# HSG-AIML/MaskedSST

Measured on NVIDIA B200. Metric: simmim_pretrain_samples_per_sec, higher is better.
Workload: dtype bf16

## Files before the change

### maskedsst_b200/csrc/attn_block_tc.cu

```cuda
#include "common.cuh"
#include "kernels.h"
#include "attn_geom.cuh"
#include "ptx.cuh"
#include <stdlib.h>
#include <stdio.h>
#include <type_traits>

namespace msst {
using namespace ptx;
typedef __nv_bfloat16 bf16;
int make_tmap_bf16_nd(CUtensorMap* m, const void* base, int rank, const int64_t* dims, const int64_t* strides, const int* box, int swizzle_bytes);
int make_tmap_nd(CUtensorMap* m, const void* base, int elem_bytes, int rank, const int64_t* dims, const int64_t* strides, const int* box, int swizzle_bytes);

namespace {

constexpr int AB_THREADS = 608;
constexpr int AB_MAXR = 8;
constexpr uint32_t AB_T16 = 16384;
constexpr uint32_t AB_BLK = 8192;
constexpr uint32_t COL_P = 0, COL_S = 192, COL_O = 256, COL_X = 192, COL_DH = 384;
constexpr uint32_t COL_Y = 320, Y_COLS = 96;

struct AbParams {
    AttnGeom g;
// ... 27 lines not shown
__device__ __forceinline__ uint64_t pair_base(const AttnGeom& g, int64_t group, int h) {
    return ((uint64_t)group * g.H + h) * (uint64_t)(TS * TS / 2);
}
__device__ __forceinline__ void group_coords(const AttnGeom& g, int64_t group, int& c1, int& c2, int& c3) {
    if (g.gpb == 0) { c1 = 0; c2 = (int)(group * g.G); c3 = 0; }
    else { c1 = (int)(group % g.gpb) * g.G; c2 = 0; c3 = (int)(group / g.gpb); }
}
__device__ __forceinline__ void store_row16(uint8_t* tile, int row, int cq, const uint32_t (&v)[16]) {
    uint8_t* r = tile + row * 128;
    const uint32_t sw = (uint32_t)(row & 7);
    *reinterpret_cast<uint4*>(r + ((((uint32_t)(2 * cq)) ^ sw) << 4)) =
        make_uint4(pack_bf(__uint_as_float(v[0]), __uint_as_float(v[1])), pack_bf(__uint_as_float(v[2]), __uint_as_float(v[3])),
                   pack_bf(__uint_as_float(v[4]), __uint_as_float(v[5])), pack_bf(__uint_as_float(v[6]), __uint_as_float(v[7])));
    *reinterpret_cast<uint4*>(r + ((((uint32_t)(2 * cq + 1)) ^ sw) << 4)) =
        make_uint4(pack_bf(__uint_as_float(v[8]), __uint_as_float(v[9])), pack_bf(__uint_as_float(v[10]), __uint_as_float(v[11])),
                   pack_bf(__uint_as_float(v[12]), __uint_as_float(v[13])), pack_bf(__uint_as_float(v[14]), __uint_as_float(v[15])));
}
__device__ __forceinline__ void store_row16_packed(uint8_t* tile, int row, int cq, const uint32_t (&pk)[8]) {
    uint8_t* r = tile + row * 128;
    const uint32_t sw = (uint32_t)(row & 7);
    *reinterpret_cast<uint4*>(r + ((((uint32_t)(2 * cq)) ^ sw) << 4)) = make_uint4(pk[0], pk[1], pk[2], pk[3]);
    *reinterpret_cast<uint4*>(r + ((((uint32_t)(2 * cq + 1)) ^ sw) << 4)) = make_uint4(pk[4], pk[5], pk[6], pk[7]);
}
__device__ __forceinline__ uint32_t key_mask16(const AttnGeom& g, int m, int cq) {
    uint32_t vm = 0;
    const int used = g.G * g.N;
    for (int j = 0; j < 16; ++j) {
        const int c = 16 * cq + j;
        const bool same = g.gpb == 0 ? (c / g.N == m / g.N) : (c % g.G == m % g.G);
        vm |= (uint32_t)(same && c < used && m < used) << j;
    }
    return vm;
}

struct alignas(8) AbBars {
    uint64_t h_full[2], h_empty[2], w_full[AB_MAXR], w_empty[AB_MAXR], do_full[2], do_empty[2];
    uint64_t pro_full, conv_done, s_full, sdp_read, p_full, o_full, a_ready, dh_full, dh_free, stg_full, stg_free, dhs_full, dhs_free;
    uint64_t y_full[2], out_full, out_free, xin_full, t_kfree[2], t_vfree[2], kv_free[2];
    uint32_t tmem_base;
};

struct AbCommon {
    uint8_t *h_s, *w_s;
    AbBars* bars;
    uint32_t tmem, h_addr, w_addr;
};
__device__ __forceinline__ void warp_arrive(uint64_t* bar, int lane) {
    __syncwarp();
    if (lane == 0) mbar_arrive(bar);
}
struct Ring {
    int slot; uint32_t ph; int NR;
    __device__ __forceinline__ void next() { if (++slot == NR) { slot = 0; ph ^= 1u; } }
};
constexpr uint64_t kDescHiK128 = ((uint64_t)(1024 >> 4) << 32) | (1ull << 46) | (kLayoutSW128 << 61);
__device__ __forceinline__ uint64_t kdesc(uint32_t addr) { return kDescHiK128 | (1ull << 16) | (uint64_t)((addr >> 4) & 0x3FFF); }
__device__ __forceinline__ uint64_t mndesc(uint32_t addr) { return kDescHiK128 | ((uint64_t)(AB_BLK >> 4) << 16) | (uint64_t)((addr >> 4) & 0x3FFF); }

template <int NCH>
__device__ __forceinline__ void load_h_tile(const AbParams& p, const CUtensorMap* tma_h, uint8_t* dst, uint64_t* bar, int64_t tile) {
    const AttnGeom& g = p.g;
    const uint32_t rows = p.nbox == 1 ? 128u : (uint32_t)(g.G * g.N);
    mbar_arrive_expect_tx(bar, (uint32_t)NCH * (uint32_t)p.nbox * rows * 64u);
    if (p.nbox == 1) {
#pragma unroll
        for (int c = 0; c < NCH; ++c) tma_load_2d(dst + c * 8192, tma_h, bar, c * 32, (int)(tile * 128));
    } else {
        for (int gi = 0; gi < 2; ++gi) {
            int c1, c2, c3;
            group_coords(g, tile * 2 + gi, c1, c2, c3);
#pragma unroll
            for (int c = 0; c < NCH; ++c) tma_load_4d(dst + c * 8192 + gi * 4096, tma_h, bar, c * 32, c1, c2, c3);
        }
    }
}
template <int NCH>
__device__ __forceinline__ void prefetch_h_tile(const AbParams& p, const CUtensorMap* tma_h, int64_t tile) {
    if (p.nbox == 1) {
#pragma unroll
        for (int c = 0; c < NCH; ++c) tma_prefetch_l2_2d(tma_h, c * 32, (int)(tile * 128));
    } else {
        for (int gi = 0; gi < 2; ++gi) {
            int c1, c2, c3;
            group_coords(p.g, tile * 2 + gi, c1, c2, c3);
#pragma unroll
            for (int c = 0; c < NCH; ++c) tma_prefetch_l2_4d(tma_h, c * 32, c1, c2, c3);
        }
    }
}
template <int NCH>
__device__ __forceinline__ void load_w_slice(const AbParams& p, const CUtensorMap* tma_w, AbBars* bars, uint8_t* w_s, Ring& r, int t, int h) {
    mbar_wait(&bars->w_empty[r.slot], r.ph ^ 1u);
    mbar_arrive_expect_tx(&bars->w_full[r.slot], (uint32_t)NCH * 4096u);
    uint8_t* dst = w_s + (size_t)r.slot * p.slot_bytes;
#pragma unroll
    for (int c = 0; c < NCH; ++c) tma_load_2d(dst + c * 4096, tma_w, &bars->w_full[r.slot], c * 32, t * p.g.H * 64 + h * 64);
    r.next();
}
template <int NCH>
__device__ __forceinline__ void issue_prologue(const AbParams& p, const AbCommon& s, int64_t k, int h, Ring& r, bool lead) {
    const int buf = (int)(k & 1);
    if (h == 0) mbar_wait(&s.bars->h_full[buf], (uint32_t)(k >> 1) & 1);
    const uint64_t ha = make_smem_desc_sw64(s.h_addr + (uint32_t)buf * p.hbuf_bytes);
    const uint32_t idesc = make_idesc_bf16(128, 64, 0, 0);
#pragma unroll
    for (int t = 0; t < 3; ++t) {
        mbar_wait(&s.bars->w_full[r.slot], r.ph);
        tc_fence_after();
        const uint64_t wa = make_smem_desc_sw64(s.w_addr + (uint32_t)r.slot * p.slot_bytes);
#pragma unroll
        for (int ks = 0; ks < 2 * NCH; ++ks)
            if (lead) umma_bf16(s.tmem + COL_P + 64 * t, ha + (uint64_t)(((ks >> 1) * 8192 + (ks & 1) * 32) >> 4), wa + (uint64_t)(((ks >> 1) * 4096 + (ks & 1) * 32) >> 4),
                      idesc, ks != 0);
        if (lead) umma_commit(&s.bars->w_empty[r.slot]);
        r.next();
    }
    if (lead && h == p.g.H - 1) umma_commit(&s.bars->h_empty[buf]);
    if (lead) umma_commit(&s.bars->pro_full);
}
template <int NCH>
__device__ __forceinline__ void issue_prologue_bwd(const AbParams& p, const AbCommon& s, int64_t k, int h, Ring& r, bool lead) {
    if (h == 0) mbar_wait(&s.bars->h_full[0], (uint32_t)k & 1);
    const uint64_t ha = make_smem_desc_sw64(s.h_addr);
    const uint32_t idesc = make_idesc_bf16(128, 64, 0, 1);
#pragma unroll
    for (int t = 0; t < 3; ++t) {
        mbar_wait(&s.bars->w_full[r.slot], r.ph);
        tc_fence_after();
        const uint64_t wa = mndesc(s.w_addr + (uint32_t)r.slot * p.slot_bytes);
#pragma unroll
        for (int ks = 0; ks < 2 * NCH; ++ks)
            if (lead) umma_bf16(s.tmem + COL_P + 64 * t, ha + (uint64_t)(((ks >> 1) * 8192 + (ks & 1) * 32) >> 4), wa + (uint64_t)(ks * 128), idesc, ks != 0);
        if (lead) umma_commit(&s.bars->w_empty[r.slot]);
        r.next();
    }
// ... 48 lines not shown
}
__device__ __forceinline__ void store_tile(const AbParams& p, const CUtensorMap* tm, const uint8_t* src, int col0, int64_t tile) {
    store_tile_rows(p, tm, src, 128, col0, tile);
}

constexpr int AB_THREADS_OUT = 736;
__device__ __forceinline__ void tail_load_x(const AbParams& p, AbBars* bars, const CUtensorMap* tma_x, uint8_t* dst, int c, int64_t tile) {
    const AttnGeom& g = p.g;
    const uint32_t rows = p.nbox == 1 ? 128u : (uint32_t)(g.G * g.N);
    mbar_arrive_expect_tx(&bars->xin_full, (uint32_t)p.nbox * rows * 128u);
    if (p.nbox == 1) tma_load_2d(dst, tma_x, &bars->xin_full, c * 32, (int)(tile * 128));
    else
        for (int gi = 0; gi < 2; ++gi) {
            int c1, c2, c3;
            group_coords(g, tile * 2 + gi, c1, c2, c3);
            tma_load_4d(dst + gi * AB_BLK, tma_x, &bars->xin_full, c * 32, c1, c2, c3);
        }
}
__device__ __forceinline__ void tail_prefetch_x(const AbParams& p, const CUtensorMap* tma_x, int c, int64_t tile) {
    if (tile >= p.n_tiles) return;
    if (p.nbox == 1) tma_prefetch_l2_2d(tma_x, c * 32, (int)(tile * 128));
    else
        for (int gi = 0; gi < 2; ++gi) {
            int c1, c2, c3;
            group_coords(p.g, tile * 2 + gi, c1, c2, c3);
            tma_prefetch_l2_4d(tma_x, c * 32, c1, c2, c3);
        }
}
__device__ __forceinline__ void tail_schedule(int h, int H, int nch, int& lo, int& hi) {
    lo = h; hi = (h == H - 1) ? nch : h;
    if (hi > nch) hi = nch;
}

template <int NCH, bool OUT>
__global__ void __launch_bounds__(OUT ? AB_THREADS_OUT : AB_THREADS, 1)
attn_block_fwd_kernel(const __grid_constant__ CUtensorMap tma_h, const __grid_constant__ CUtensorMap tma_w, const __grid_constant__ CUtensorMap tma_o,
                      const __grid_constant__ CUtensorMap tma_wo, const __grid_constant__ CUtensorMap tma_xmid, const __grid_constant__ CUtensorMap tma_h2,
                      const __grid_constant__ CUtensorMap tma_x, const __grid_constant__ AbParams p) {
    extern __shared__ __align__(1024) uint8_t smem_raw[];
    uint8_t* smem = smem_raw;
    if (smem_u32(smem) & 1023u) __trap();
    const AttnGeom& g = p.g;
    AbCommon s;
    s.h_s = smem; s.w_s = s.h_s + 2 * p.hbuf_bytes;
    uint8_t* qkv_s = s.w_s + (size_t)p.NR * p.slot_bytes;
    uint8_t* p_s = qkv_s + 6 * AB_T16;
    float* xch = reinterpret_cast<float*>(p_s + AB_T16);
    s.bars = reinterpret_cast<AbBars*>(xch + 2 * 4 * 128);
    AbBars* bars = s.bars;
    const int warp = threadIdx.x >> 5;
    const int H = g.H;
    constexpr int D = NCH * 32;
    ab_setup(bars, warp, s.h_s, 2 * p.hbuf_bytes, nullptr, 0, &tma_h, &tma_w, &tma_o, OUT ? &tma_wo : nullptr, OUT ? &tma_xmid : nullptr, OUT ? 2u : 1u);
    s.tmem = bars->tmem_base; s.h_addr = smem_u32(s.h_s); s.w_addr = smem_u32(s.w_s);

    const int64_t my_tiles = blockIdx.x < p.n_tiles ? (p.n_tiles - 1 - blockIdx.x) / gridDim.x + 1 : 0;
    const int64_t n_items = my_tiles * H;
    if (warp < 16) {
        const int lq = warp & 3, cq = warp >> 2, lane = threadIdx.x & 31;
        const int L = lq * 32 + lane;
        const uint32_t lane_addr = (uint32_t)(lq * 32) << 16;
        const int slot = 64 * ((lane >> 4) & 1) + 16 * lq + (lane & 15);
        const int blk = slot >> 6, m = slot & 63;
        const float sl2 = g.scale * 1.4426950408889634f;
        const bool full_blocks = g.N == 64 && g.groups % 2 == 0;
        const uint64_t seed = p.drop.seed + (p.drop.seed_dev ? __ldg(p.drop.seed_dev) : 0ull);
        const uint32_t t16 = p.drop.thresh >> 16;
        const uint32_t vm_geom = full_blocks ? 0xFFFFu : key_mask16(g, m, cq);
        float* xmax = xch; float* xsum = xch + 4 * 128;
        int64_t cur_tile = -1, grow = -1; uint32_t vm = 0;
        int64_t k = 0; int h = 0;
        bool hosted = false; uint32_t n_kvf0 = 0, n_kvf1 = 0;
        if (n_items > 0) {
            mbar_wait(&bars->pro_full, 0);
            tc_fence_after();
            convert_qkv(s.tmem, qkv_s, lane_addr, L, cq);
            tc_fence_before();
            fence_proxy_async();
            warp_arrive(&bars->conv_done, lane);
        }
        for (int64_t it = 0; it < n_items; ++it) {
            const uint32_t ph = (uint32_t)it & 1;
            const int64_t tile = blockIdx.x + k * gridDim.x;
            if (tile != cur_tile) {
                cur_tile = tile;
                int64_t seq; int pos;
                const int64_t group = tile * 2 + blk;
                const bool ok = group < g.groups && slot_to(g, group, 0, m, seq, pos);
                grow = ok ? row_of(g, seq, pos) : -1;
                vm = ok ? vm_geom : 0u;
            }
            const uint64_t hidx = pair_base(g, tile * 2 + blk, h) + (uint64_t)(m * 32 + 8 * cq);
            const uint32_t hash_lo = (uint32_t)hidx + (uint32_t)(seed >> 32);
            const uint32_t hash_hi = ((uint32_t)(hidx >> 32) * 0x85EBCA77u) ^ (uint32_t)seed ^ (p.drop.site * 0xC2B2AE3Du);
            if (threadIdx.x == 0) AB_T(it, 0);
            mbar_wait(&bars->s_full, ph);
            if (threadIdx.x == 0) AB_T(it, 1);
            tc_fence_after();
            float sc[16];
            {
                uint32_t a[16];
                tmem_ld_32x16(s.tmem + lane_addr + COL_S + 16 * cq, a);
                tmem_ld_wait();
#pragma unroll
                for (int j = 0; j < 16; ++j) sc[j] = __uint_as_float(a[j]);
            }
            float mx = -INFINITY;
            if (vm == 0xFFFFu) {
#pragma unroll
                for (int j = 0; j < 16; ++j) mx = fmaxf(mx, sc[j]);
            } else {
#pragma unroll
                for (int j = 0; j < 16; ++j) { sc[j] = (vm >> j) & 1u ? sc[j] : -INFINITY; mx = fmaxf(mx, sc[j]); }
            }
            xmax[cq * 128 + L] = mx;
            asm volatile("bar.sync 1, 512;" ::: "memory");
            mx = fmaxf(fmaxf(xmax[L], xmax[128 + L]), fmaxf(xmax[256 + L], xmax[384 + L]));
            const float sub = mx == -INFINITY ? 0.f : mx * sl2;
            float l = 0.f;
            uint32_t pk[8];
            auto exp_row = [&](auto drop_tag) {
                constexpr bool DROP = decltype(drop_tag)::value;
#pragma unroll
                for (int jj = 0; jj < 8; ++jj) {
                    float p0 = ex2_approx(fmaf(sc[2 * jj], sl2, -sub)), p1 = ex2_approx(fmaf(sc[2 * jj + 1], sl2, -sub));
                    l += p0 + p1;
                    if (DROP) {
                        uint32_t x = (hash_lo + (uint32_t)jj) * 0x9E3779B1u ^ hash_hi;
                        x ^= x >> 16; x *= 0x7feb352du; x ^= x >> 15; x *= 0x846ca68bu; x ^= x >> 16;
                        p0 *= (x & 0xFFFFu) >= t16 ? p.drop.scale : 0.f;
                        p1 *= (x >> 16) >= t16 ? p.drop.scale : 0.f;
                    }
                    pk[jj] = pack_bf(p0, p1);
                }
            };
            if (p.drop.on()) exp_row(std::true_type{}); else exp_row(std::false_type{});
            xsum[cq * 128 + L] = l;
            store_row16_packed(p_s + blk * AB_BLK, m, cq, pk);
            fence_proxy_async();
            tc_fence_before();
            warp_arrive(&bars->p_full, lane);
            if (threadIdx.x == 0) AB_T(it, 2);
            asm volatile("bar.sync 1, 512;" ::: "memory");
            l = (xsum[L] + xsum[128 + L]) + (xsum[256 + L] + xsum[384 + L]);
            const float inv = l > 0.f ? 1.f / l : 0.f;
            if (cq == 0 && grow >= 0) p.lse_out[grow * H + h] = (sub + log2f(l)) * 0.6931471805599453f;
            if (it >= 1) mbar_wait(&bars->stg_free, (uint32_t)(it - 1) & 1);
            if (it + 1 < n_items) {
                if (OUT && hosted) {
                    if (it & 1) { mbar_wait(&bars->kv_free[0], n_kvf0 & 1u); ++n_kvf0; }
                    else { mbar_wait(&bars->kv_free[1], n_kvf1 & 1u); ++n_kvf1; }
                }
                mbar_wait(&bars->pro_full, ph ^ 1u);
                if (threadIdx.x == 0) AB_T(it, 3);
                tc_fence_after();
                convert_qkv(s.tmem, qkv_s + (size_t)((it + 1) & 1) * 3 * AB_T16, lane_addr, L, cq);
                tc_fence_before();
                fence_proxy_async();
                warp_arrive(&bars->conv_done, lane);
                if (threadIdx.x == 0) AB_T(it, 4);
            }
            mbar_wait(&bars->o_full, ph);
            if (threadIdx.x == 0) AB_T(it, 5);
            tc_fence_after();
            {
                uint32_t v[16], o8[8];
                tmem_ld_32x16(s.tmem + lane_addr + COL_O + 16 * cq, v);
                tmem_ld_wait();
#pragma unroll
                for (int j = 0; j < 8; ++j) o8[j] = pack_bf(__uint_as_float(v[2 * j]) * inv, __uint_as_float(v[2 * j + 1]) * inv);
                store_row16_packed(qkv_s + (size_t)(it & 1) * 3 * AB_T16, slot, cq, o8);
            }
            tc_fence_before();
            fence_proxy_async();
            warp_arrive(&bars->stg_full, lane);
            if (threadIdx.x == 0) AB_T(it, 6);
            if (OUT) { int lo, hi; tail_schedule(h, H, NCH, lo, hi); hosted = k > 0 && lo <= hi; }
            if (++h == H) { h = 0; ++k; }
        }
    } else
    if (warp >= 16 && warp < 19) {
    if (warp == 16) {
        if (elect_one()) {
            Ring r{0, 0u, p.NR};
            int64_t pk = 0; int phd = 0;
            auto load_pro = [&]() {
                if (phd == 0) {
                    const int buf = (int)(pk & 1);
                    mbar_wait(&bars->h_empty[buf], ((uint32_t)(pk >> 1) & 1) ^ 1);
                    load_h_tile<NCH>(p, &tma_h, s.h_s + (size_t)buf * p.hbuf_bytes, &bars->h_full[buf], blockIdx.x + pk * gridDim.x);
                }
                for (int t = 0; t < 3; ++t) load_w_slice<NCH>(p, &tma_w, bars, s.w_s, r, t, phd);
                if (++phd == H) { phd = 0; ++pk; }
            };
            int yh = 0;
            auto load_wo = [&]() {
                mbar_wait(&bars->w_empty[r.slot], r.ph ^ 1u);
                mbar_arrive_expect_tx(&bars->w_full[r.slot], (uint32_t)D * 128u);
                tma_load_2d(s.w_s + (size_t)r.slot * p.slot_bytes, &tma_wo, &bars->w_full[r.slot], yh * 64, 0);
                r.next();
                if (++yh == H) yh = 0;
            };
            if (n_items > 0) load_pro();
            if (n_items > 1) load_pro();
            for (int64_t it = 0; it < n_items; ++it) {
                if (OUT && it >= 1) load_wo();
                if (it + 2 < n_items) load_pro();
            }
            if (OUT && n_items > 0) load_wo();
        }
    } else if (warp == 17) {
        if (n_items > 0) {
            const bool lead = elect_one();
            Ring r{0, 0u, p.NR};
            const uint32_t idesc_s = make_idesc_bf16(64, 64, 0, 0), idesc_o = make_idesc_bf16(64, 64, 0, 1), idesc_y = make_idesc_bf16(128, D, 0, 0);
            const uint32_t qkv_addr = smem_u32(qkv_s);
            const uint64_t pd0 = kdesc(smem_u32(p_s)), pd1 = kdesc(smem_u32(p_s) + AB_BLK);
            int64_t pk = 0; int phd = 0;
            auto next_pro = [&]() { issue_prologue<NCH>(p, s, pk, phd, r, lead); if (++phd == H) { phd = 0; ++pk; } };
            int64_t sk = 0; int sh = 0;
            auto issue_s = [&](int64_t it) {
                const uint32_t qa = qkv_addr + (uint32_t)(it & 1) * 3 * AB_T16;
                mbar_wait(&bars->conv_done, (uint32_t)it & 1);
                if (lead) AB_T(it, 8);
                tc_fence_after();
#pragma unroll
                for (int b = 0; b < 2; ++b) {
                    const uint64_t dq = kdesc(qa + b * AB_BLK), dk = kdesc(qa + AB_T16 + b * AB_BLK);
#pragma unroll
                    for (int ks = 0; ks < 4; ++ks)
                        if (lead) umma_bf16(s.tmem + COL_S + ((uint32_t)(16 * b) << 16), dq + (uint64_t)(ks * 2), dk + (uint64_t)(ks * 2), idesc_s, ks != 0);
                }
                if (lead) umma_commit(&bars->s_full);
                if (OUT) {
                    int lo, hi;
                    tail_schedule(sh, H, NCH, lo, hi);
                    if (lead && sk > 0 && lo <= hi) umma_commit(&bars->t_kfree[it & 1]);
                    if (++sh == H) { sh = 0; ++sk; }
                }
            };
            int yh = 0; uint32_t ycol = COL_Y;
            auto issue_y = [&](int64_t it) {
                mbar_wait(&bars->stg_full, (uint32_t)it & 1);
                mbar_wait(&bars->w_full[r.slot], r.ph);
                if (lead) AB_T(it, 11);
                tc_fence_after();
                const uint64_t ad = kdesc(qkv_addr + (uint32_t)(it & 1) * 3 * AB_T16), bd = kdesc(s.w_addr + (uint32_t)r.slot * p.slot_bytes);
#pragma unroll
                for (int ks = 0; ks < 4; ++ks)
                    if (lead && !(p.tail_dbg & 1)) umma_bf16(s.tmem + ycol, ad + (uint64_t)(ks * 2), bd + (uint64_t)(ks * 2), idesc_y, (yh | ks) != 0);
                if (lead) {
                    umma_commit(&bars->w_empty[r.slot]);
// ... 172 lines not shown
#pragma unroll 1
                    for (int i = 0; i < D / 16; ++i) {
                        uint32_t a[16];
                        tmem_ld_32x16(ty + 16 * i, a);
                        tmem_ld_wait();
                        const int col = 16 * i;
#pragma unroll
                        for (int u = 0; u < 2; ++u) {
                            uint32_t o[4];
#pragma unroll
                            for (int hf = 0; hf < 2; ++hf) {
                                const int e0 = 8 * u + 4 * hf;
                                const float4 w = *reinterpret_cast<const float4*>(cst + D + col + e0), lb = *reinterpret_cast<const float4*>(cst + 2 * D + col + e0);
                                o[2 * hf] = pack_bf((__uint_as_float(a[e0]) - mean) * rstd * w.x + lb.x, (__uint_as_float(a[e0 + 1]) - mean) * rstd * w.y + lb.y);
                                o[2 * hf + 1] = pack_bf((__uint_as_float(a[e0 + 2]) - mean) * rstd * w.z + lb.z, (__uint_as_float(a[e0 + 3]) - mean) * rstd * w.w + lb.w);
                            }
                            *reinterpret_cast<uint4*>(kv + (i >> 1) * 8192 + T * 64 + ((((uint32_t)(2 * (i & 1) + u)) ^ sw64) << 4)) = make_uint4(o[0], o[1], o[2], o[3]);
                        }
                    }
                }
                tc_fence_before();
                fence_proxy_async();
                warp_arrive(&bars->out_full, lane);
                ++n_out;
                if (T == 0 && !last) AB_T(host, 15);
            }
        }
    }
    tc_fence_before();
    __syncthreads();
    if (warp == 16) { tc_fence_after(); tmem_dealloc(s.tmem, 512); }
}

template <int NCH>
__global__ void __launch_bounds__(AB_THREADS, 1)
attn_block_bwd_kernel(const __grid_constant__ CUtensorMap tma_h, const __grid_constant__ CUtensorMap tma_wt, const __grid_constant__ CUtensorMap tma_do,
                      const __grid_constant__ CUtensorMap tma_dqkv, const __grid_constant__ CUtensorMap tma_dh, const AbParams p) {
    extern __shared__ __align__(1024) uint8_t smem_raw[];
    uint8_t* smem = smem_raw;
    if (smem_u32(smem) & 1023u) __trap();
    const AttnGeom& g = p.g;
    AbCommon s;
    s.h_s = smem; s.w_s = s.h_s + p.hbuf_bytes;
    uint8_t* qkv_s = s.w_s + (size_t)p.NR * p.slot_bytes;
    uint8_t* do_s = qkv_s + 3 * AB_T16;
    uint8_t* p_s = do_s + 2 * AB_T16;
    uint8_t* ds_s = p_s + AB_T16;
    uint8_t* dhs_s = ds_s + AB_T16;
    float* xch = reinterpret_cast<float*>(dhs_s + AB_T16);
    s.bars = reinterpret_cast<AbBars*>(xch + 4 * 128);
    AbBars* bars = s.bars;
    const int warp = threadIdx.x >> 5;
    const int H = g.H, I = H * 64;
    constexpr int D = NCH * 32;
    ab_setup(bars, warp, s.h_s, p.hbuf_bytes, do_s, 2 * AB_T16, &tma_h, &tma_wt, &tma_do, &tma_dqkv, &tma_dh);
    s.tmem = bars->tmem_base; s.h_addr = smem_u32(s.h_s); s.w_addr = smem_u32(s.w_s);

    const int64_t my_tiles = blockIdx.x < p.n_tiles ? (p.n_tiles - 1 - blockIdx.x) / gridDim.x + 1 : 0;
    const int64_t n_items = my_tiles * H;
    const uint32_t do_rows = p.nbox == 1 ? 128u : (uint32_t)(g.G * g.N);

    if (warp == 16) {
        if (elect_one()) {
            Ring r{0, 0u, p.NR};
            auto load_do = [&](int64_t it, int64_t tile, int h) {
                const int st = (int)(it & 1);
                mbar_wait(&bars->do_empty[st], ((uint32_t)(it >> 1) & 1) ^ 1);
// ... 132 lines not shown
                const int64_t tile = blockIdx.x + (it / H) * gridDim.x; const int h = (int)(it % H);
                const int st = (int)(it & 1);
                mbar_wait(&bars->stg_full, (uint32_t)it & 1);
                store_tile(p, &tma_dqkv, p_s, h * 64, tile);
                store_tile(p, &tma_dqkv, ds_s, I + h * 64, tile);
                store_tile(p, &tma_dqkv, do_s + (size_t)st * AB_T16, 2 * I + h * 64, tile);
                tma_store_commit();
                tma_store_wait_read();
                mbar_arrive(&bars->stg_free);
                mbar_arrive(&bars->do_empty[st]);
                if (h == H - 1) {
                    const int64_t rd0 = (it / H) * NCH;
                    for (int c = 0; c < NCH; ++c) {
                        mbar_wait(&bars->dhs_full, (uint32_t)(rd0 + c) & 1);
                        store_tile(p, &tma_dh, dhs_s, 32 * c, tile);
                        tma_store_commit();
                        tma_store_wait_read();
                        mbar_arrive(&bars->dhs_free);
                    }
                }
            }
        }
    } else {
        const int lq = warp & 3, cq = warp >> 2, lane = threadIdx.x & 31;
        const int L = lq * 32 + lane;
        const uint32_t lane_addr = (uint32_t)(lq * 32) << 16;
        const int slot = 64 * ((lane >> 4) & 1) + 16 * lq + (lane & 15);
        const int blk = slot >> 6, m = slot & 63;
        const float sl2 = g.scale * 1.4426950408889634f;
        const bool full_blocks = g.N == 64 && g.groups % 2 == 0;
        const uint64_t seed = p.drop.seed + (p.drop.seed_dev ? __ldg(p.drop.seed_dev) : 0ull);
        const uint32_t t16 = p.drop.thresh >> 16;
        const uint32_t vm_geom = full_blocks ? 0xFFFFu : key_mask16(g, m, cq);
        struct Item { int64_t k, tile, grow; int h; uint32_t vm; };
        auto locate = [&](Item& x) {
            int64_t seq; int pos;
            const int64_t group = x.tile * 2 + blk;
            const bool ok = group < g.groups && slot_to(g, group, 0, m, seq, pos);
            x.grow = ok ? row_of(g, seq, pos) : -1;
            x.vm = ok ? vm_geom : 0u;
        };
        auto advance = [&](Item& x) {
            if (++x.h == H) { x.h = 0; ++x.k; x.tile = blockIdx.x + x.k * gridDim.x; locate(x); }
        };
        auto convert = [&](int64_t it) {
            mbar_wait(&bars->pro_full, (uint32_t)it & 1);
            if (threadIdx.x == 0) AB_T(it, 1);
            tc_fence_after();
            convert_qkv(s.tmem, qkv_s, lane_addr, L, cq);
            tc_fence_before();
            fence_proxy_async();
            warp_arrive(&bars->conv_done, lane);
            if (threadIdx.x == 0) AB_T(it, 2);
        };
        auto softmax = [&](int64_t it, const Item& x) {
            const float Lse = x.grow >= 0 ? __ldg(p.lse_in + x.grow * H + x.h) * 1.4426950408889634f : 0.f;
            const uint64_t hidx = pair_base(g, x.tile * 2 + blk, x.h) + (uint64_t)(m * 32 + 8 * cq);
            const uint32_t hash_lo = (uint32_t)hidx + (uint32_t)(seed >> 32);
            const uint32_t hash_hi = ((uint32_t)(hidx >> 32) * 0x85EBCA77u) ^ (uint32_t)seed ^ (p.drop.site * 0xC2B2AE3Du);
            const uint32_t vm = x.vm;
            mbar_wait(&bars->s_full, (uint32_t)it & 1);
            if (threadIdx.x == 0) AB_T(it, 3);
            tc_fence_after();
            float sp[16], dp[16];
            {
                uint32_t a[16], b[16];
                tmem_ld_32x16(s.tmem + lane_addr + COL_P + 16 * cq, a);
                tmem_ld_32x16(s.tmem + lane_addr + COL_P + 64 + 16 * cq, b);
                tmem_ld_wait();
                tc_fence_before();
                warp_arrive(&bars->sdp_read, lane);
#pragma unroll
                for (int j = 0; j < 16; ++j) { sp[j] = __uint_as_float(a[j]); dp[j] = __uint_as_float(b[j]); }
            }
            uint32_t pk[8], dk[8];
            float D0 = 0.f, D1 = 0.f;
#pragma unroll
            for (int jj = 0; jj < 8; ++jj) {
                const int j = 2 * jj;
                float f0 = 1.f, f1 = 1.f;
                if (p.drop.on()) {
                    uint32_t y = (hash_lo + (uint32_t)jj) * 0x9E3779B1u ^ hash_hi;
                    y ^= y >> 16; y *= 0x7feb352du; y ^= y >> 15; y *= 0x846ca68bu; y ^= y >> 16;
                    f0 = (y & 0xFFFFu) >= t16 ? p.drop.scale : 0.f;
                    f1 = (y >> 16) >= t16 ? p.drop.scale : 0.f;
                }
                float p0 = ex2_approx(fmaf(sp[j], sl2, -Lse)), p1 = ex2_approx(fmaf(sp[j + 1], sl2, -Lse));
                if (vm != 0xFFFFu) {
                    p0 = (vm >> j) & 1u ? p0 : 0.f;
                    p1 = (vm >> (j + 1)) & 1u ? p1 : 0.f;
                }
                const float pf0 = p0 * f0, pf1 = p1 * f1;
                D0 = fmaf(pf0, dp[j], D0); D1 = fmaf(pf1, dp[j + 1], D1);
                pk[jj] = pack_bf(pf0, pf1);
                sp[j] = p0 * g.scale; sp[j + 1] = p1 * g.scale;
                dp[j] *= f0; dp[j + 1] *= f1;
            }
            xch[cq * 128 + L] = D0 + D1;
            asm volatile("bar.sync 1, 512;" ::: "memory");
            const float Dp = (xch[L] + xch[128 + L]) + (xch[256 + L] + xch[384 + L]);
#pragma unroll
            for (int jj = 0; jj < 8; ++jj) dk[jj] = pack_bf(sp[2 * jj] * (dp[2 * jj] - Dp), sp[2 * jj + 1] * (dp[2 * jj + 1] - Dp));
            if (it >= 1) mbar_wait(&bars->stg_free, (uint32_t)(it - 1) & 1);
            store_row16_packed(p_s + blk * AB_BLK, m, cq, pk);
            store_row16_packed(ds_s + blk * AB_BLK, m, cq, dk);
            fence_proxy_async();
            tc_fence_before();
// ... 73 lines not shown
    }
    if (g.gpb == 0) {
        const int64_t dims[4] = {cols, g.N, g.n_seq, 1}, strides[3] = {cols, (int64_t)g.N * cols, g.n_seq * g.N * cols};
        const int box[4] = {box_cols, g.N, g.G, 1};
        return make_tmap_nd(m, base, elem_bytes, 4, dims, strides, box, swizzle);
    }
    const int64_t dims[4] = {cols, g.inner, g.N, g.n_seq / g.inner};
    const int64_t strides[3] = {cols, (int64_t)g.inner * cols, (int64_t)g.N * g.inner * cols};
    const int box[4] = {box_cols, g.G, g.N, 1};
    return make_tmap_nd(m, base, elem_bytes, 4, dims, strides, box, swizzle);
}

long long* g_dbg = nullptr;
int dbg_level() {
    static int v = -1;
    if (v < 0) { const char* e = getenv("MSST_AB_DBG"); v = e ? atoi(e) : 0; if (v) cudaMalloc(&g_dbg, 48 * 16 * 8); }
    return v;
}
void dbg_dump(const char* what, cudaStream_t st, int& count) {
    if (++count != dbg_level()) return;
    static long long h[48 * 16];
    cudaStreamSynchronize(st);
    cudaMemcpy(h, g_dbg, sizeof(h), cudaMemcpyDeviceToHost);
    const long long t0 = h[0];
    printf("%s timeline, CTA 0 (clks rel. to item 0), compute slots 0-6 | MMA-issuer slots 8-12 (see the AB_T calls)\n", what);
    for (int i = 0; i < 40; ++i) {
        printf("%2d:", i);
        for (int k = 0; k < 16; ++k) { if (k == 7) { printf("  |"); continue; } printf(" %7lld", h[i * 16 + k] ? h[i * 16 + k] - t0 : -1); }
        printf("\n");
    }
    fflush(stdout);
}

int fill_params(AbParams& p, const AttnGeom& g, int D, bool bwd, size_t& smem_bytes) {
    p.g = g; p.D = D; p.nch = D / 32;
    p.dbg = dbg_level() ? g_dbg : nullptr;
    p.nbox = (g.gpb == 0 && g.G * g.N == 64) ? 1 : 2;
    p.n_tiles = (g.groups + 1) / 2;
    p.slot_bytes = (uint32_t)D * 128u;
    p.hbuf_bytes = (uint32_t)p.nch * 8192u;
    p.hbufs = bwd ? 1 : 2;
    const size_t fixed = (size_t)p.hbufs * p.hbuf_bytes + (bwd ? 8 * AB_T16 + 4 * 128 * sizeof(float) : 7 * AB_T16 + 2 * 4 * 128 * sizeof(float)) + sizeof(AbBars) +
                         (bwd ? 0 : 16 + 3 * 96 * sizeof(float));
    const size_t cap = 232448;
    int nr = AB_MAXR;
    const int nr_min = bwd ? 6 : 3;
    while (nr > nr_min && fixed + (size_t)nr * p.slot_bytes > cap) --nr;
    MSST_REQUIRE(fixed + (size_t)nr * p.slot_bytes <= cap, "attn_block: D = %d does not fit shared memory", D);
    p.NR = nr;
    smem_bytes = fixed + (size_t)nr * p.slot_bytes;
    return MSST_OK;
}

}

bool attn_block_supported(const AttnGeom& g, int D) {
    return attention_bwd_tc_supported(g) && g.dh == 64 && D % 32 == 0 && D >= 32 && D <= 96 && g.H * 64 * 3 < 65536;
}

template <int NCH, bool OUT>
static int launch_fwd(const CUtensorMap& t_h, const CUtensorMap& t_w, const CUtensorMap& t_o, const CUtensorMap& t_wo, const CUtensorMap& t_xmid,
                      const CUtensorMap& t_h2, const CUtensorMap& t_x, const AbParams& p, int grid, size_t smem, cudaStream_t st) {
    static PerDeviceOnce once;
    if (once.first()) MSST_CUDA(cudaFuncSetAttribute(attn_block_fwd_kernel<NCH, OUT>, cudaFuncAttributeMaxDynamicSharedMemorySize, 232448));
    attn_block_fwd_kernel<NCH, OUT><<<grid, OUT ? AB_THREADS_OUT : AB_THREADS, smem, st>>>(t_h, t_w, t_o, t_wo, t_xmid, t_h2, t_x, p);
    return MSST_OK;
}

int attn_block_fwd(const AttnGeom& g, int D, const bf16* h, const bf16* w_qkv, bf16* out, float* lse, Drop drop, cudaStream_t st, const AttnBlockOut* tail) {
    MSST_REQUIRE(attn_block_supported(g, D), "attn_block_fwd: needs packed short sequences (N <= 64), dim_head 64, D in {32, 64, 96}");
    AbParams p{};
    size_t smem = 0;
    if (int rc = fill_params(p, g, D, false, smem)) return rc;
    p.lse_out = lse; p.o = out; p.drop = drop;
    CUtensorMap t_h, t_w, t_o, t_wo, t_xmid, t_h2, t_x;
    const int64_t I = (int64_t)g.H * 64;
    if (int rc = act_tmap(&t_h, g, h, D, p.nbox, 32, 64)) return rc;
    if (out) { if (int rc = act_tmap(&t_o, g, out, I, p.nbox, 64, 128)) return rc; }
    else t_o = t_h;
    const int64_t I3 = I * 3;
    { const int64_t dims[2] = {D, I3}, strides[1] = {D}; const int box[2] = {32, 64};
      if (int rc = make_tmap_bf16_nd(&t_w, w_qkv, 2, dims, strides, box, 64)) return rc; }
    if (tail) {
        MSST_REQUIRE(g.n_seq * g.N < (int64_t)2147483647, "attn_block_fwd: the fused out-projection indexes rows with 32 bits");
        MSST_REQUIRE(tail->w_out && tail->b_out && tail->x && tail->xmid && tail->ln_w && tail->ln_b && tail->h2 && tail->ln_stats,
                     "attn_block_fwd: the fused out-projection needs w_out, b_out, x, xmid, ln_w, ln_b, h2 and ln_stats");
        p.x_res = tail->x; p.b_out = tail->b_out; p.ln_w = tail->ln_w; p.ln_b = tail->ln_b; p.ln_stats = tail->ln_stats; p.drop_out = tail->drop;
        { static int v = -1; if (v < 0) { const char* e = getenv("MSST_AB_TAILDBG"); v = e ? atoi(e) : 0; } p.tail_dbg = v; }
        { const int64_t dims[2] = {I, D}, strides[1] = {I}; const int box[2] = {64, D};
          if (int rc = make_tmap_bf16_nd(&t_wo, tail->w_out, 2, dims, strides, box, 128)) return rc; }
        if (int rc = act_tmap(&t_xmid, g, tail->xmid, D, p.nbox, 32, 128, 4)) return rc;
        if (int rc = act_tmap(&t_x, g, tail->x, D, p.nbox, 32, 128, 4)) return rc;
        if (int rc = act_tmap(&t_h2, g, tail->h2, D, p.nbox, 32, 64)) return rc;
    } else {
        MSST_REQUIRE(out, "attn_block_fwd: null output");
        t_wo = t_h; t_xmid = t_h; t_h2 = t_h; t_x = t_h;
    }
    const int grid = (int)(p.n_tiles < kNumSMs ? p.n_tiles : kNumSMs);
    if (p.dbg) cudaMemsetAsync(p.dbg, 0, 48 * 16 * 8, st);
    int rc = MSST_OK;
    switch (p.nch * 2 + (tail ? 1 : 0)) {
        case 2: rc = launch_fwd<1, false>(t_h, t_w, t_o, t_wo, t_xmid, t_h2, t_x, p, grid, smem, st); break;
        case 3: rc = launch_fwd<1, true>(t_h, t_w, t_o, t_wo, t_xmid, t_h2, t_x, p, grid, smem, st); break;
        case 4: rc = launch_fwd<2, false>(t_h, t_w, t_o, t_wo, t_xmid, t_h2, t_x, p, grid, smem, st); break;
        case 5: rc = launch_fwd<2, true>(t_h, t_w, t_o, t_wo, t_xmid, t_h2, t_x, p, grid, smem, st); break;
        case 6: rc = launch_fwd<3, false>(t_h, t_w, t_o, t_wo, t_xmid, t_h2, t_x, p, grid, smem, st); break;
        default: rc = launch_fwd<3, true>(t_h, t_w, t_o, t_wo, t_xmid, t_h2, t_x, p, grid, smem, st); break;
    }
    if (rc) return rc;
    MSST_LAUNCH_CHECK();
    if (p.dbg) { static int n = 0; dbg_dump("attn_block_fwd", st, n); }
    return MSST_OK;
}

int attn_block_bwd(const AttnGeom& g, int D, const bf16* h, const bf16* w_qkv, const bf16* w_qkv_t, const bf16* d_out, const float* lse,
                   bf16* d_qkv, float* d_h, Drop drop, cudaStream_t st) {
    MSST_REQUIRE(attn_block_supported(g, D), "attn_block_bwd: needs packed short sequences (N <= 64), dim_head 64, D in {32, 64, 96}");
    AbParams p{};
    size_t smem = 0;
    if (int rc = fill_params(p, g, D, true, smem)) return rc;
    p.lse_in = lse; p.dqkv = d_qkv; p.dh = d_h; p.drop = drop;
    static PerDeviceOnce once;
    if (once.first()) {
        MSST_CUDA(cudaFuncSetAttribute(attn_block_bwd_kernel<1>, cudaFuncAttributeMaxDynamicSharedMemorySize, 232448));
        MSST_CUDA(cudaFuncSetAttribute(attn_block_bwd_kernel<2>, cudaFuncAttributeMaxDynamicSharedMemorySize, 232448));
        MSST_CUDA(cudaFuncSetAttribute(attn_block_bwd_kernel<3>, cudaFuncAttributeMaxDynamicSharedMemorySize, 232448));
    }
    CUtensorMap t_h, t_wt, t_do, t_dqkv, t_dh;
    (void)w_qkv;
    const int64_t I = (int64_t)g.H * 64, I3 = 3 * I;
    if (int rc = act_tmap(&t_h, g, h, D, p.nbox, 32, 64)) return rc;
    if (int rc = act_tmap(&t_do, g, d_out, I, p.nbox, 64, 128)) return rc;
    if (int rc = act_tmap(&t_dqkv, g, d_qkv, I3, p.nbox, 64, 128)) return rc;
    if (int rc = act_tmap(&t_dh, g, d_h, D, p.nbox, 32, 128, 4)) return rc;
    { const int64_t dims[2] = {I3, D}, strides[1] = {I3}; const int box[2] = {64, D};
      if (int rc = make_tmap_bf16_nd(&t_wt, w_qkv_t, 2, dims, strides, box, 128)) return rc; }
    const int grid = (int)(p.n_tiles < kNumSMs ? p.n_tiles : kNumSMs);
    if (p.dbg) cudaMemsetAsync(p.dbg, 0, 48 * 16 * 8, st);
    switch (p.nch) {
        case 1: attn_block_bwd_kernel<1><<<grid, AB_THREADS, smem, st>>>(t_h, t_wt, t_do, t_dqkv, t_dh, p); break;
        case 2: attn_block_bwd_kernel<2><<<grid, AB_THREADS, smem, st>>>(t_h, t_wt, t_do, t_dqkv, t_dh, p); break;
        default: attn_block_bwd_kernel<3><<<grid, AB_THREADS, smem, st>>>(t_h, t_wt, t_do, t_dqkv, t_dh, p); break;
    }
    MSST_LAUNCH_CHECK();
    if (p.dbg) { static int n = 0; dbg_dump("attn_block_bwd", st, n); }
    return MSST_OK;
}

}
```

Baseline: 62940.

## Process only real key columns in strided-group attention softmax paths

When keys are grouped by stride with many groups (gpb>0, G>=8), each row's 16-column chunk holds only about two valid keys. The new KS=2 specialisation precomputes those column indices once and runs exp, dropout hashing and bf16 stores only for them, in both the forward and backward softmax epilogues. The backward path zero-fills the P and dS tiles before scattering the few real values. To make room, the forward kernel drops to a single H buffer in this mode, which may reduce load/compute overlap.

```diff
diff --git a/maskedsst_b200/csrc/attn_block_tc.cu b/maskedsst_b200/csrc/attn_block_tc.cu
--- a/maskedsst_b200/csrc/attn_block_tc.cu
+++ b/maskedsst_b200/csrc/attn_block_tc.cu
@@ -83,6 +83,45 @@
     }
     return vm;
 }
+template <int KS>
+__host__ __device__ constexpr int lo_col(int i) { return (16 * i + KS - 1) / KS; }
+template <int KS>
+struct RealCols {
+    int j[KS];
+    uint32_t off[KS];
+    uint32_t on;
+};
+template <int KS>
+__device__ __forceinline__ RealCols<KS> real_cols(uint32_t vm, int row, int cq) {
+    RealCols<KS> r;
+    r.on = 0;
+#pragma unroll
+    for (int i = 0; i < KS; ++i) {
+        r.j[i] = vm ? __ffs(vm) - 1 : lo_col<KS>(i);
+        r.on |= (uint32_t)(vm != 0) << i;
+        vm &= vm - 1;
+        r.off[i] = ((((uint32_t)(2 * cq + (r.j[i] >> 3))) ^ (uint32_t)(row & 7)) << 4) + 2u * (uint32_t)(r.j[i] & 7);
+    }
+    return r;
+}
+__device__ __forceinline__ float pick16(const float (&v)[16], int j, int lo) {
+    float a[8], b[4], c[2];
+#pragma unroll
+    for (int i = 0; i < 8; ++i) a[i] = (j & 1) ? v[2 * i + 1 < lo ? lo : 2 * i + 1] : v[2 * i < lo ? lo : 2 * i];
+#pragma unroll
+    for (int i = 0; i < 4; ++i) b[i] = (j & 2) ? a[2 * i + 1] : a[2 * i];
+#pragma unroll
+    for (int i = 0; i < 2; ++i) c[i] = (j & 4) ? b[2 * i + 1] : b[2 * i];
+    return (j & 8) ? c[1] : c[0];
+}
+__device__ __forceinline__ bool drop_keep(uint32_t hash_lo, uint32_t hash_hi, int j, uint32_t t16) {
+    uint32_t x = (hash_lo + (uint32_t)(j >> 1)) * 0x9E3779B1u ^ hash_hi;
+    x ^= x >> 16; x *= 0x7feb352du; x ^= x >> 15; x *= 0x846ca68bu; x ^= x >> 16;
+    return ((j & 1) ? x >> 16 : x & 0xFFFFu) >= t16;
+}
+__device__ __forceinline__ void store_bf16(uint8_t* tile, int row, uint32_t off, float v) {
+    *reinterpret_cast<__nv_bfloat16*>(tile + row * 128 + off) = __float2bfloat16_rn(v);
+}
 
 struct alignas(8) AbBars {
     uint64_t h_full[2], h_empty[2], w_full[AB_MAXR], w_empty[AB_MAXR], do_full[2], do_empty[2];
@@ -148,10 +187,10 @@
     for (int c = 0; c < NCH; ++c) tma_load_2d(dst + c * 4096, tma_w, &bars->w_full[r.slot], c * 32, t * p.g.H * 64 + h * 64);
     r.next();
 }
-template <int NCH>
+template <int NCH, int HB>
 __device__ __forceinline__ void issue_prologue(const AbParams& p, const AbCommon& s, int64_t k, int h, Ring& r, bool lead) {
-    const int buf = (int)(k & 1);
-    if (h == 0) mbar_wait(&s.bars->h_full[buf], (uint32_t)(k >> 1) & 1);
+    const int buf = HB == 2 ? (int)(k & 1) : 0;
+    if (h == 0) mbar_wait(&s.bars->h_full[buf], HB == 2 ? (uint32_t)(k >> 1) & 1 : (uint32_t)k & 1);
     const uint64_t ha = make_smem_desc_sw64(s.h_addr + (uint32_t)buf * p.hbuf_bytes);
     const uint32_t idesc = make_idesc_bf16(128, 64, 0, 0);
 #pragma unroll
@@ -266,7 +305,7 @@
     if (hi > nch) hi = nch;
 }
 
-template <int NCH, bool OUT>
+template <int NCH, bool OUT, int KS>
 __global__ void __launch_bounds__(OUT ? AB_THREADS_OUT : AB_THREADS, 1)
 attn_block_fwd_kernel(const __grid_constant__ CUtensorMap tma_h, const __grid_constant__ CUtensorMap tma_w, const __grid_constant__ CUtensorMap tma_o,
                       const __grid_constant__ CUtensorMap tma_wo, const __grid_constant__ CUtensorMap tma_xmid, const __grid_constant__ CUtensorMap tma_h2,
@@ -276,7 +315,8 @@
     if (smem_u32(smem) & 1023u) __trap();
     const AttnGeom& g = p.g;
     AbCommon s;
-    s.h_s = smem; s.w_s = s.h_s + 2 * p.hbuf_bytes;
+    constexpr int HB = KS ? 1 : 2;
+    s.h_s = smem; s.w_s = s.h_s + HB * p.hbuf_bytes;
     uint8_t* qkv_s = s.w_s + (size_t)p.NR * p.slot_bytes;
     uint8_t* p_s = qkv_s + 6 * AB_T16;
     float* xch = reinterpret_cast<float*>(p_s + AB_T16);
@@ -285,7 +325,7 @@
     const int warp = threadIdx.x >> 5;
     const int H = g.H;
     constexpr int D = NCH * 32;
-    ab_setup(bars, warp, s.h_s, 2 * p.hbuf_bytes, nullptr, 0, &tma_h, &tma_w, &tma_o, OUT ? &tma_wo : nullptr, OUT ? &tma_xmid : nullptr, OUT ? 2u : 1u);
+    ab_setup(bars, warp, s.h_s, HB * p.hbuf_bytes, KS ? p_s : nullptr, KS ? AB_T16 : 0u, &tma_h, &tma_w, &tma_o, OUT ? &tma_wo : nullptr, OUT ? &tma_xmid : nullptr, OUT ? 2u : 1u);
     s.tmem = bars->tmem_base; s.h_addr = smem_u32(s.h_s); s.w_addr = smem_u32(s.w_s);
 
     const int64_t my_tiles = blockIdx.x < p.n_tiles ? (p.n_tiles - 1 - blockIdx.x) / gridDim.x + 1 : 0;
@@ -301,6 +341,7 @@
         const uint64_t seed = p.drop.seed + (p.drop.seed_dev ? __ldg(p.drop.seed_dev) : 0ull);
         const uint32_t t16 = p.drop.thresh >> 16;
         const uint32_t vm_geom = full_blocks ? 0xFFFFu : key_mask16(g, m, cq);
+        const RealCols<KS ? KS : 1> rc = real_cols<KS ? KS : 1>(vm_geom, m, cq);
         float* xmax = xch; float* xsum = xch + 4 * 128;
         int64_t cur_tile = -1, grow = -1; uint32_t vm = 0;
         int64_t k = 0; int h = 0;
@@ -322,7 +363,7 @@
                 const int64_t group = tile * 2 + blk;
                 const bool ok = group < g.groups && slot_to(g, group, 0, m, seq, pos);
                 grow = ok ? row_of(g, seq, pos) : -1;
-                vm = ok ? vm_geom : 0u;
+                vm = ok ? (KS ? rc.on : vm_geom) : 0u;
             }
             const uint64_t hidx = pair_base(g, tile * 2 + blk, h) + (uint64_t)(m * 32 + 8 * cq);
             const uint32_t hash_lo = (uint32_t)hidx + (uint32_t)(seed >> 32);
@@ -340,7 +381,11 @@
                 for (int j = 0; j < 16; ++j) sc[j] = __uint_as_float(a[j]);
             }
             float mx = -INFINITY;
-            if (vm == 0xFFFFu) {
+            float sv[KS ? KS : 1];
+            if constexpr (KS > 0) {
+#pragma unroll
+                for (int i = 0; i < KS; ++i) { sv[i] = (vm >> i) & 1u ? pick16(sc, rc.j[i], lo_col<KS>(i)) : -INFINITY; mx = fmaxf(mx, sv[i]); }
+            } else if (vm == 0xFFFFu) {
 #pragma unroll
                 for (int j = 0; j < 16; ++j) mx = fmaxf(mx, sc[j]);
             } else {
@@ -353,6 +398,16 @@
             const float sub = mx == -INFINITY ? 0.f : mx * sl2;
             float l = 0.f;
             uint32_t pk[8];
+            auto exp_cols = [&](auto drop_tag) {
+                constexpr bool DROP = decltype(drop_tag)::value;
+#pragma unroll
+                for (int i = 0; i < KS; ++i) {
+                    float pv = ex2_approx(fmaf(sv[i], sl2, -sub));
+                    l += pv;
+                    if (DROP) pv *= drop_keep(hash_lo, hash_hi, rc.j[i], t16) ? p.drop.scale : 0.f;
+                    if ((rc.on >> i) & 1u) store_bf16(p_s + blk * AB_BLK, m, rc.off[i], pv);
+                }
+            };
             auto exp_row = [&](auto drop_tag) {
                 constexpr bool DROP = decltype(drop_tag)::value;
 #pragma unroll
@@ -368,9 +423,13 @@
                     pk[jj] = pack_bf(p0, p1);
                 }
             };
-            if (p.drop.on()) exp_row(std::true_type{}); else exp_row(std::false_type{});
+            if constexpr (KS > 0) {
+                if (p.drop.on()) exp_cols(std::true_type{}); else exp_cols(std::false_type{});
+            } else {
+                if (p.drop.on()) exp_row(std::true_type{}); else exp_row(std::false_type{});
+                store_row16_packed(p_s + blk * AB_BLK, m, cq, pk);
+            }
             xsum[cq * 128 + L] = l;
-            store_row16_packed(p_s + blk * AB_BLK, m, cq, pk);
             fence_proxy_async();
             tc_fence_before();
             warp_arrive(&bars->p_full, lane);
@@ -420,8 +479,8 @@
             int64_t pk = 0; int phd = 0;
             auto load_pro = [&]() {
                 if (phd == 0) {
-                    const int buf = (int)(pk & 1);
-                    mbar_wait(&bars->h_empty[buf], ((uint32_t)(pk >> 1) & 1) ^ 1);
+                    const int buf = HB == 2 ? (int)(pk & 1) : 0;
+                    mbar_wait(&bars->h_empty[buf], (HB == 2 ? (uint32_t)(pk >> 1) & 1 : (uint32_t)pk & 1) ^ 1);
                     load_h_tile<NCH>(p, &tma_h, s.h_s + (size_t)buf * p.hbuf_bytes, &bars->h_full[buf], blockIdx.x + pk * gridDim.x);
                 }
                 for (int t = 0; t < 3; ++t) load_w_slice<NCH>(p, &tma_w, bars, s.w_s, r, t, phd);
@@ -451,7 +510,7 @@
             const uint32_t qkv_addr = smem_u32(qkv_s);
             const uint64_t pd0 = kdesc(smem_u32(p_s)), pd1 = kdesc(smem_u32(p_s) + AB_BLK);
             int64_t pk = 0; int phd = 0;
-            auto next_pro = [&]() { issue_prologue<NCH>(p, s, pk, phd, r, lead); if (++phd == H) { phd = 0; ++pk; } };
+            auto next_pro = [&]() { issue_prologue<NCH, HB>(p, s, pk, phd, r, lead); if (++phd == H) { phd = 0; ++pk; } };
             int64_t sk = 0; int sh = 0;
             auto issue_s = [&](int64_t it) {
                 const uint32_t qa = qkv_addr + (uint32_t)(it & 1) * 3 * AB_T16;
@@ -690,7 +749,7 @@
     if (warp == 16) { tc_fence_after(); tmem_dealloc(s.tmem, 512); }
 }
 
-template <int NCH>
+template <int NCH, int KS>
 __global__ void __launch_bounds__(AB_THREADS, 1)
 attn_block_bwd_kernel(const __grid_constant__ CUtensorMap tma_h, const __grid_constant__ CUtensorMap tma_wt, const __grid_constant__ CUtensorMap tma_do,
                       const __grid_constant__ CUtensorMap tma_dqkv, const __grid_constant__ CUtensorMap tma_dh, const AbParams p) {
@@ -889,13 +948,14 @@
         const uint64_t seed = p.drop.seed + (p.drop.seed_dev ? __ldg(p.drop.seed_dev) : 0ull);
         const uint32_t t16 = p.drop.thresh >> 16;
         const uint32_t vm_geom = full_blocks ? 0xFFFFu : key_mask16(g, m, cq);
+        const RealCols<KS ? KS : 1> rc = real_cols<KS ? KS : 1>(vm_geom, m, cq);
         struct Item { int64_t k, tile, grow; int h; uint32_t vm; };
         auto locate = [&](Item& x) {
             int64_t seq; int pos;
             const int64_t group = x.tile * 2 + blk;
             const bool ok = group < g.groups && slot_to(g, group, 0, m, seq, pos);
             x.grow = ok ? row_of(g, seq, pos) : -1;
-            x.vm = ok ? vm_geom : 0u;
+            x.vm = ok ? (KS ? rc.on : vm_geom) : 0u;
         };
         auto advance = [&](Item& x) {
             if (++x.h == H) { x.h = 0; ++x.k; x.tile = blockIdx.x + x.k * gridDim.x; locate(x); }
@@ -930,6 +990,40 @@
 #pragma unroll
                 for (int j = 0; j < 16; ++j) { sp[j] = __uint_as_float(a[j]); dp[j] = __uint_as_float(b[j]); }
             }
+            if constexpr (KS > 0) {
+                float pf[KS], ps[KS], dd[KS];
+                float D0 = 0.f, D1 = 0.f;
+#pragma unroll
+                for (int i = 0; i < KS; ++i) {
+                    const int j = rc.j[i];
+                    const float f = p.drop.on() ? (drop_keep(hash_lo, hash_hi, j, t16) ? p.drop.scale : 0.f) : 1.f;
+                    float p0 = ex2_approx(fmaf(pick16(sp, j, lo_col<KS>(i)), sl2, -Lse));
+                    p0 = (vm >> i) & 1u ? p0 : 0.f;
+                    const float d = pick16(dp, j, lo_col<KS>(i));
+                    pf[i] = p0 * f;
+                    const float t = fmaf(pf[i], d, (j & 1) ? D1 : D0);
+                    if (j & 1) D1 = t; else D0 = t;
+                    ps[i] = p0 * g.scale; dd[i] = d * f;
+                }
+                xch[cq * 128 + L] = D0 + D1;
+                asm volatile("bar.sync 1, 512;" ::: "memory");
+                const float Dp = (xch[L] + xch[128 + L]) + (xch[256 + L] + xch[384 + L]);
+                if (it >= 1) mbar_wait(&bars->stg_free, (uint32_t)(it - 1) & 1);
+                const uint32_t zero[8] = {0u, 0u, 0u, 0u, 0u, 0u, 0u, 0u};
+                store_row16_packed(p_s + blk * AB_BLK, m, cq, zero);
+                store_row16_packed(ds_s + blk * AB_BLK, m, cq, zero);
+#pragma unroll
+                for (int i = 0; i < KS; ++i)
+                    if ((rc.on >> i) & 1u) {
+                        store_bf16(p_s + blk * AB_BLK, m, rc.off[i], pf[i]);
+                        store_bf16(ds_s + blk * AB_BLK, m, rc.off[i], ps[i] * (dd[i] - Dp));
+                    }
+                fence_proxy_async();
+                tc_fence_before();
+                warp_arrive(&bars->p_full, lane);
+                if (threadIdx.x == 0) AB_T(it, 4);
+                return;
+            }
             uint32_t pk[8], dk[8];
             float D0 = 0.f, D1 = 0.f;
 #pragma unroll
@@ -1069,6 +1163,8 @@
     fflush(stdout);
 }
 
+static int sparse_keys(const AttnGeom& g) { return g.gpb > 0 && g.G >= 8 ? 2 : 0; }
+
 int fill_params(AbParams& p, const AttnGeom& g, int D, bool bwd, size_t& smem_bytes) {
     p.g = g; p.D = D; p.nch = D / 32;
     p.dbg = dbg_level() ? g_dbg : nullptr;
@@ -1076,7 +1172,7 @@
     p.n_tiles = (g.groups + 1) / 2;
     p.slot_bytes = (uint32_t)D * 128u;
     p.hbuf_bytes = (uint32_t)p.nch * 8192u;
-    p.hbufs = bwd ? 1 : 2;
+    p.hbufs = bwd || sparse_keys(g) ? 1 : 2;
     const size_t fixed = (size_t)p.hbufs * p.hbuf_bytes + (bwd ? 8 * AB_T16 + 4 * 128 * sizeof(float) : 7 * AB_T16 + 2 * 4 * 128 * sizeof(float)) + sizeof(AbBars) +
                          (bwd ? 0 : 16 + 3 * 96 * sizeof(float));
     const size_t cap = 232448;
@@ -1098,9 +1194,11 @@
 template <int NCH, bool OUT>
 static int launch_fwd(const CUtensorMap& t_h, const CUtensorMap& t_w, const CUtensorMap& t_o, const CUtensorMap& t_wo, const CUtensorMap& t_xmid,
                       const CUtensorMap& t_h2, const CUtensorMap& t_x, const AbParams& p, int grid, size_t smem, cudaStream_t st) {
-    static PerDeviceOnce once;
-    if (once.first()) MSST_CUDA(cudaFuncSetAttribute(attn_block_fwd_kernel<NCH, OUT>, cudaFuncAttributeMaxDynamicSharedMemorySize, 232448));
-    attn_block_fwd_kernel<NCH, OUT><<<grid, OUT ? AB_THREADS_OUT : AB_THREADS, smem, st>>>(t_h, t_w, t_o, t_wo, t_xmid, t_h2, t_x, p);
+    const int sparse = sparse_keys(p.g) ? 1 : 0;
+    auto kern = sparse ? attn_block_fwd_kernel<NCH, OUT, 2> : attn_block_fwd_kernel<NCH, OUT, 0>;
+    static PerDeviceOnce once[2];
+    if (once[sparse].first()) MSST_CUDA(cudaFuncSetAttribute(kern, cudaFuncAttributeMaxDynamicSharedMemorySize, 232448));
+    kern<<<grid, OUT ? AB_THREADS_OUT : AB_THREADS, smem, st>>>(t_h, t_w, t_o, t_wo, t_xmid, t_h2, t_x, p);
     return MSST_OK;
 }
 
@@ -1159,9 +1257,12 @@
     p.lse_in = lse; p.dqkv = d_qkv; p.dh = d_h; p.drop = drop;
     static PerDeviceOnce once;
     if (once.first()) {
-        MSST_CUDA(cudaFuncSetAttribute(attn_block_bwd_kernel<1>, cudaFuncAttributeMaxDynamicSharedMemorySize, 232448));
-        MSST_CUDA(cudaFuncSetAttribute(attn_block_bwd_kernel<2>, cudaFuncAttributeMaxDynamicSharedMemorySize, 232448));
-        MSST_CUDA(cudaFuncSetAttribute(attn_block_bwd_kernel<3>, cudaFuncAttributeMaxDynamicSharedMemorySize, 232448));
+        MSST_CUDA(cudaFuncSetAttribute(attn_block_bwd_kernel<1, 0>, cudaFuncAttributeMaxDynamicSharedMemorySize, 232448));
+        MSST_CUDA(cudaFuncSetAttribute(attn_block_bwd_kernel<2, 0>, cudaFuncAttributeMaxDynamicSharedMemorySize, 232448));
+        MSST_CUDA(cudaFuncSetAttribute(attn_block_bwd_kernel<3, 0>, cudaFuncAttributeMaxDynamicSharedMemorySize, 232448));
+        MSST_CUDA(cudaFuncSetAttribute(attn_block_bwd_kernel<1, 2>, cudaFuncAttributeMaxDynamicSharedMemorySize, 232448));
+        MSST_CUDA(cudaFuncSetAttribute(attn_block_bwd_kernel<2, 2>, cudaFuncAttributeMaxDynamicSharedMemorySize, 232448));
+        MSST_CUDA(cudaFuncSetAttribute(attn_block_bwd_kernel<3, 2>, cudaFuncAttributeMaxDynamicSharedMemorySize, 232448));
     }
     CUtensorMap t_h, t_wt, t_do, t_dqkv, t_dh;
     (void)w_qkv;
@@ -1174,11 +1275,11 @@
       if (int rc = make_tmap_bf16_nd(&t_wt, w_qkv_t, 2, dims, strides, box, 128)) return rc; }
     const int grid = (int)(p.n_tiles < kNumSMs ? p.n_tiles : kNumSMs);
     if (p.dbg) cudaMemsetAsync(p.dbg, 0, 48 * 16 * 8, st);
-    switch (p.nch) {
-        case 1: attn_block_bwd_kernel<1><<<grid, AB_THREADS, smem, st>>>(t_h, t_wt, t_do, t_dqkv, t_dh, p); break;
-        case 2: attn_block_bwd_kernel<2><<<grid, AB_THREADS, smem, st>>>(t_h, t_wt, t_do, t_dqkv, t_dh, p); break;
-        default: attn_block_bwd_kernel<3><<<grid, AB_THREADS, smem, st>>>(t_h, t_wt, t_do, t_dqkv, t_dh, p); break;
-    }
+    const bool sparse = sparse_keys(g) != 0;
+    auto kern = p.nch == 1 ? (sparse ? attn_block_bwd_kernel<1, 2> : attn_block_bwd_kernel<1, 0>)
+              : p.nch == 2 ? (sparse ? attn_block_bwd_kernel<2, 2> : attn_block_bwd_kernel<2, 0>)
+                           : (sparse ? attn_block_bwd_kernel<3, 2> : attn_block_bwd_kernel<3, 0>);
+    kern<<<grid, AB_THREADS, smem, st>>>(t_h, t_wt, t_do, t_dqkv, t_dh, p);
     MSST_LAUNCH_CHECK();
     if (p.dbg) { static int n = 0; dbg_dump("attn_block_bwd", st, n); }
     return MSST_OK;
diff --git a/profiles/dump_attn_block.py b/profiles/dump_attn_block.py
--- /dev/null
+++ b/profiles/dump_attn_block.py
@@ -0,0 +1,73 @@
+import argparse
+import ctypes as C
+import os
+import sys
+
+import torch
+
+sys.path.insert(0, os.path.dirname(os.path.dirname(os.path.abspath(__file__))))
+
+STACKS = {"spatial": lambda B, Cb: (B * Cb, 64, 1), "spectral": lambda B, Cb: (B * 64, Cb, 64)}
+
+
+def dump(out_dir, B=1024, Cb=5, H=8, D=96, drop=0.1):
+    from maskedsst_b200 import _lib
+    lib = _lib.lib()
+    st = torch.cuda.current_stream().cuda_stream
+    os.makedirs(out_dir, exist_ok=True)
+    R, I = B * Cb * 64, H * 64
+    for name, shape in STACKS.items():
+        n_seq, N, inner = shape(B, Cb)
+        g = torch.Generator(device="cuda").manual_seed(1234)
+        rnd = lambda *s: torch.randn(*s, device="cuda", generator=g)
+        h = rnd(R, D).bfloat16()
+        w = (rnd(3 * I, D) * D ** -0.5).bfloat16()
+        wt = w.t().contiguous()
+        w_out = (rnd(D, I) * I ** -0.5).bfloat16()
+        b_out, x, ln_w, ln_b = rnd(D), rnd(R, D), 1 + 0.2 * rnd(D), 0.2 * rnd(D)
+        do = rnd(R, I).bfloat16()
+        o = torch.empty(R, I, device="cuda", dtype=torch.bfloat16)
+        lse = torch.empty(R, H, device="cuda")
+        xmid = torch.empty(R, D, device="cuda")
+        h2 = torch.empty(R, D, device="cuda", dtype=torch.bfloat16)
+        stats2 = torch.empty(R, 2, device="cuda")
+        dqkv = torch.empty(R, 3 * I, device="cuda", dtype=torch.bfloat16)
+        dh = torch.empty(R, D, device="cuda")
+        ad = _lib.AttnDims(n_seq, N, inner, H, 64, drop, 1234, 16, _lib.PREC_BF16, None)
+        _lib.check(lib.msst_attn_block_out_fwd(C.byref(ad), D, h.data_ptr(), w.data_ptr(), o.data_ptr(), lse.data_ptr(), w_out.data_ptr(),
+                                               b_out.data_ptr(), x.data_ptr(), xmid.data_ptr(), ln_w.data_ptr(), ln_b.data_ptr(),
+                                               h2.data_ptr(), stats2.data_ptr(), 17, st))
+        _lib.check(lib.msst_attn_block_bwd(C.byref(ad), D, h.data_ptr(), w.data_ptr(), wt.data_ptr(), do.data_ptr(), lse.data_ptr(),
+                                           dqkv.data_ptr(), dh.data_ptr(), st))
+        torch.cuda.synchronize()
+        torch.save({k: v.cpu() for k, v in dict(o=o, lse=lse, xmid=xmid, h2=h2, stats2=stats2, dqkv=dqkv, dh=dh).items()},
+                   os.path.join(out_dir, f"{name}.pt"))
+        print(f"{name}: n_seq {n_seq} N {N} inner {inner} -> {out_dir}/{name}.pt", flush=True)
+
+
+def compare(a_dir, b_dir):
+    same = True
+    for name in STACKS:
+        a, b = torch.load(os.path.join(a_dir, f"{name}.pt")), torch.load(os.path.join(b_dir, f"{name}.pt"))
+        for k in a:
+            ta, tb = a[k], b[k]
+            if torch.equal(ta.view(torch.int16) if ta.dtype == torch.bfloat16 else ta.view(torch.int32),
+                           tb.view(torch.int16) if tb.dtype == torch.bfloat16 else tb.view(torch.int32)):
+                print(f"{name:8s} {k:6s} bit-equal")
+                continue
+            same = False
+            fa, fb = ta.double(), tb.double()
+            rel = ((fa - fb).abs().max() / fa.abs().max().clamp_min(1e-30)).item()
+            print(f"{name:8s} {k:6s} DIFFERS: {(ta != tb).sum().item()} elements, max |a - b| / max |a| = {rel:.3e}")
+    print("all outputs bit-equal" if same else "outputs differ")
+    return same
+
+
+if __name__ == "__main__":
+    ap = argparse.ArgumentParser()
+    ap.add_argument("--out")
+    ap.add_argument("--compare", nargs=2)
+    args = ap.parse_args()
+    if args.compare:
+        sys.exit(0 if compare(*args.compare) else 1)
+    dump(args.out)
```

Result: faster. 64070 (median of 6 runs) (+1.8%).
